# pashtari/lrf

Hardware: AMD Instinct MI355X
Metric: Mpixels/sec qmf_encode (8x8 patch, r=7, 10 iters) (higher is better)
Workload: dtype f32; 1 GPU; 256 x 512x768x3 uint8 per GPU, YCbCr 4:2:0, 8x8 patches, ranks (7,3,3), bounds (-16,15), num_iters 10, int8 factors out (BASELINE configs[1]); priming_steps=3, global_batch=256, rank_input_bytes=301989888, parallelism=images sharded over 1 GPU(s), no data-path collective

## Files before the change

lrf_amd/csrc/lrf_bcd_persist.hip:

```cpp
#include "lrf_host.h"
#include "lrf_gs.h"
#include "lrf_bcdw_kernel.hip"
#include "lrf_bcdw16_kernel.hip"
#include "lrf_bcdw32_kernel.hip"
#include "lrf_bcdp_kernel.hip"

PersistPlan bcdp_plan(lrf_ctx* c, const std::vector<FamRun>& runs, int K, int lo, int hi)
{
    PersistPlan pp;
    static const int persist_env = (int)env_long("LRF_PERSIST", -1);
    static const bool exact_off = dev_flag("LRF_GENERIC_GS");
    if (!c->persist_arch || persist_env == 0 || !bcd_wave_variant() || K < 2 || runs.empty()) return pp;
    const long mx = abs(lo) > abs(hi) ? abs(lo) : abs(hi);
    long nblocks = 0;
    bool f16 = false;
    int np32 = 0;
    for (const FamRun& r : runs) {
        if (fam_of_rank(r.rmin) != r.fam || fam_of_rank(r.rmax) != r.fam) return pp;
        nblocks += r.nblocks;
        if (r.fam == 0) continue;
        const bool exact = !exact_off && (long)(r.rmax - 1) * 64 * mx * mx * mx < (1L << 24);
        if (!exact || r.any_native) return pp;
        if (r.fam == 1) {
            f16 = true;
        } else {
            const int np = (r.rmax + 1) >> 1;
            if (64 * mx * mx > 32767 || r.rmin < 2 * np - 1 || (np32 != 0 && np32 != np)) return pp;
            np32 = np;
        }
    }
    const long min_blocks = runs.size() == 1 ? LRF_PERSIST_MIN_BLOCKS_ONE_FAMILY : LRF_PERSIST_MIN_BLOCKS;
    if (nblocks < (persist_env == 1 ? LRF_BCDW_MIN_BLOCKS : min_blocks)) return pp;
    pp.use = true;
    pp.f16 = f16 || np32 != 0;
    pp.np32 = np32;
    static const bool first_off = dev_flag("LRF_NO_PERSIST_FIRST");
    pp.first = np32 == 0 && !first_off;
    return pp;
}

template <bool F16, int NP32, bool FIRST = false>
static int bcdp_launch_t(lrf_ctx* c, int attr_bit, int wgs, int wave_lds, const float* X, const PlaneDesc* pl, const BlockDesc* bl, int nblocks,
                         int nplanes, int plane0, const BcdpTabs& t16, const BcdpTabs& t64, int8_t* U, int8_t* V, GsParams gp, int niter)
{
    if (!(c->attr_persist & (1u << attr_bit))) {
        HIP_TRY(hipFuncSetAttribute((const void*)k_bcd_p<F16, NP32, FIRST>, hipFuncAttributeMaxDynamicSharedMemorySize, LRF_BCDW_WAVES * wave_lds));
        c->attr_persist |= 1u << attr_bit;
    }
    Prof p(c, LRF_K_BCD_PERSIST);
    hipLaunchKernelGGL((k_bcd_p<F16, NP32, FIRST>), dim3((unsigned)wgs), dim3(64 * LRF_BCDW_WAVES), (size_t)LRF_BCDW_WAVES * wave_lds, c->stream, X, pl, bl, t16,
                       t64, U, V, gp, nblocks, niter, nplanes, plane0, (BcdpSync*)c->psync.p, c->h_perr, 2 * nplanes, ++c->pseq, wave_lds);
    LAUNCH_CHECK();
    return LRF_OK;
}

int bcdp_launch(lrf_ctx* c, const PersistPlan& pp, const float* X, const PlaneDesc* pl, const BlockDesc* bl, int nblocks, int nplanes, int plane0,
                const FamBufs& f16, const FamBufs& f64, int8_t* U, int8_t* V, GsParams gp, int niter, bool first)
{
    if (first && (!pp.first || pp.np32 != 0)) return set_err(LRF_EINVAL, "internal: first iteration inside k_bcd_p with ranks above 16");
    if (!c->h_perr) {
        HIP_TRY(hipHostMalloc((void**)&c->h_perr, sizeof(int), hipHostMallocDefault));
        *c->h_perr = 0;
    }
    int rc = ctx_check(c);
    if (rc) return rc;
    const size_t sbytes = sizeof(BcdpSync) + (2 * (size_t)nplanes + (size_t)nblocks) * sizeof(int);
    const void* before = c->psync.p;
    if ((rc = ensure(c, c->psync, sbytes))) return rc;
    if (c->psync.p != before || c->psync_dirty) {
        HIP_TRY(hipMemsetAsync(c->psync.p, 0, c->psync.cap, c->stream));
        c->psync_dirty = false;
    }
    const long total_waves = (long)niter * nblocks;
    long wgs = (total_waves + LRF_BCDW_WAVES - 1) / LRF_BCDW_WAVES;
    if (wgs > 512) wgs = 512;
    int wave_lds = (64 * 64 + 64 * 8) * 4;
    if (pp.f16 && LRF_BCDW16_WAVE_LDS > wave_lds) wave_lds = LRF_BCDW16_WAVE_LDS;
    const BcdpTabs t16{f16.vf, f16.bf, f16.pp, f16.qp, f16.wf}, t64{f64.vf, f64.bf, f64.pp, f64.qp, f64.wf};
    gp.exact_int = 1;
#define LRF_P(F16, NP, BIT)                                                                                                          \
    return bcdp_launch_t<F16, NP>(c, BIT, (int)wgs, NP ? (LRF_BCDW32_WAVE_LDS(NP) > wave_lds ? LRF_BCDW32_WAVE_LDS(NP) : wave_lds) : wave_lds, X, pl, bl, \
                                  nblocks, nplanes, plane0, t16, t64, U, V, gp, niter)
    if (first) {
        if (!pp.f16) return bcdp_launch_t<false, 0, true>(c, 10, (int)wgs, wave_lds, X, pl, bl, nblocks, nplanes, plane0, t16, t64, U, V, gp, niter);
        return bcdp_launch_t<true, 0, true>(c, 11, (int)wgs, wave_lds, X, pl, bl, nblocks, nplanes, plane0, t16, t64, U, V, gp, niter);
    }
    if (!pp.f16) LRF_P(false, 0, 0);
    switch (pp.np32) {
    case 0: LRF_P(true, 0, 1);
    case 9: LRF_P(true, 9, 2);
    case 10: LRF_P(true, 10, 3);
    case 11: LRF_P(true, 11, 4);
    case 12: LRF_P(true, 12, 5);
    case 13: LRF_P(true, 13, 6);
    case 14: LRF_P(true, 14, 7);
    case 15: LRF_P(true, 15, 8);
    default: LRF_P(true, 16, 9);
    }
#undef LRF_P
}
```

lrf_amd/csrc/lrf_bcdp_kernel.hip:

```cpp
#pragma once

#ifndef LRF_BCDP_MAX_POLLS
#define LRF_BCDP_MAX_POLLS (1 << 20)
#endif

struct BcdpSync {
    int head;
    int done;
    int err;
    int pad[29];
    int cell[1];
};

struct BcdpTabs {
    float *vf, *bf, *pp, *qp;
    const float* wf;
};

__device__ __forceinline__ float ld_sc1(const float* p) { return __hip_atomic_load(p, __ATOMIC_RELAXED, __HIP_MEMORY_SCOPE_AGENT); }
__device__ __forceinline__ void st_sc1(float* p, float v)
{
#ifdef LRF_BCDP_PLAIN_PSTORE
    *p = v;
#else
    __hip_atomic_store(p, v, __ATOMIC_RELAXED, __HIP_MEMORY_SCOPE_AGENT);
#endif
}
__device__ __forceinline__ void st_sc1_u32_unaligned(void* p, unsigned v)
{
#ifdef LRF_BCDP_PLAIN_USTORE
    *reinterpret_cast<u32_unaligned*>(p) = v;
#else
    asm volatile("global_store_dword %0, %1, off sc1" ::"v"(p), "v"(v) : "memory");
#endif
}
__device__ __forceinline__ unsigned ld_sc1_u32_unaligned(const void* p)
{
    unsigned v;
    asm volatile("global_load_dword %0, %1, off sc1" : "=v"(v) : "v"(p) : "memory");
    return v;
}

__device__ __forceinline__ void bcdp_sum16(const PlaneDesc& pd, const float* __restrict__ Ppart, const float* __restrict__ Qpart, int lane,
                                           float (&acc)[16], float (&q)[4])
{
#pragma unroll
    for (int j = 0; j < 16; j++) acc[j] = 0.f;
#pragma unroll
    for (int j = 0; j < 4; j++) q[j] = 0.f;
    const float* Pp = Ppart + (long)pd.blk0 * 64 * LRF_RP + lane;
    const float* Qp = Qpart + (long)pd.blk0 * LRF_RP * LRF_RP + lane;
    constexpr int NB = 4;
    for (int b0 = 0; b0 < pd.nblk; b0 += NB) {
        float pv[NB][16], qv[NB][4];
#pragma unroll
        for (int k = 0; k < NB; k++) {
            const long blk = b0 + k < pd.nblk ? b0 + k : b0;
#pragma unroll
            for (int j = 0; j < 16; j++) pv[k][j] = ld_sc1(Pp + blk * 64 * LRF_RP + 64 * j);
#pragma unroll
            for (int j = 0; j < 4; j++) qv[k][j] = ld_sc1(Qp + blk * LRF_RP * LRF_RP + 64 * j);
        }
#pragma unroll
        for (int k = 0; k < NB; k++)
            if (b0 + k < pd.nblk) {
#pragma unroll
                for (int j = 0; j < 16; j++) acc[j] = (b0 + k == 0) ? pv[k][j] : acc[j] + pv[k][j];
#pragma unroll
                for (int j = 0; j < 4; j++) q[j] = (b0 + k == 0) ? qv[k][j] : q[j] + qv[k][j];
            }
    }
}
__device__ __forceinline__ void bcdp_wave_sync()
{
    __builtin_amdgcn_fence(__ATOMIC_RELEASE, "wavefront");
    __builtin_amdgcn_wave_barrier();
    __builtin_amdgcn_fence(__ATOMIC_ACQUIRE, "wavefront");
}

__device__ __forceinline__ void bcdp_vupdate(const PlaneDesc& pd, int pli, const float* __restrict__ Ppart, const float* __restrict__ Qpart,
                                             float* __restrict__ Vf, float* __restrict__ Bf, int8_t* __restrict__ V8, const GsParams gp,
                                             int write_i8, float* lds, int lane)
{
    float* a_s = lds;
    float* v_s = lds + 64 * LRF_RP;
    float* gt_s = lds + 2 * 64 * LRF_RP;
    const int R = pd.R;
    float acc[16], q[4];
    bcdp_sum16(pd, Ppart, Qpart, lane, acc, q);
#pragma unroll
    for (int j = 0; j < 16; j++) {
        a_s[lane + 64 * j] = acc[j];
        v_s[lane + 64 * j] = ld_sc1(Vf + (long)pli * 64 * LRF_RP + lane + 64 * j);
    }
#pragma unroll
    for (int j = 0; j < 4; j++) {
        const int idx = lane + 64 * j, jj = idx >> 4, r = idx & 15;
        if (jj < R && r < R) {
            if (jj == r) {
                const float den = (q[j] + 0.f) + LRF_EPS;
                gt_s[r * LRF_GT_LD + LRF_GT_DEN] = den;
                gt_s[r * LRF_GT_LD + LRF_GT_RDEN] = 1.0f / den;
            } else {
                gt_s[r * LRF_GT_LD + (jj < r ? jj : jj - 1)] = q[j];
            }
        }
    }
    __builtin_amdgcn_fence(__ATOMIC_RELEASE, "wavefront");
    __builtin_amdgcn_wave_barrier();
    __builtin_amdgcn_fence(__ATOMIC_ACQUIRE, "wavefront");
    {
        const bool native = (long)(R - 1) * 64 < 400;
        const float no_tab[17] = {0.f, 0.f, 0.f, 0.f, 0.f, 0.f, 0.f, 0.f, 0.f, 0.f, 0.f, 0.f, 0.f, 0.f, 0.f, 0.f, 0.f};
        gs_dispatch<8, false>(R, &a_s[lane * LRF_RP], &v_s[lane * LRF_RP], nullptr, 0, gt_s, native, gp, no_tab);
        float* Vp = Vf + (long)pli * 64 * LRF_RP + lane * LRF_RP;
        for (int r = 0; r < R; r++) st_sc1(Vp + r, v_s[lane * LRF_RP + r]);
        if (write_i8) {
            int8_t* vo = V8 + pd.v_off + (long)lane * R;
            for (int r = 0; r < R; r++) vo[r] = (int8_t)v_s[lane * LRF_RP + r];
        }
    }
    __builtin_amdgcn_fence(__ATOMIC_RELEASE, "wavefront");
    __builtin_amdgcn_wave_barrier();
    __builtin_amdgcn_fence(__ATOMIC_ACQUIRE, "wavefront");
    if (!write_i8) {
        float* gt_n = a_s;
        make_gtable(v_s, 64, R, gt_n, lane, 64);
        __builtin_amdgcn_fence(__ATOMIC_RELEASE, "wavefront");
        __builtin_amdgcn_wave_barrier();
        __builtin_amdgcn_fence(__ATOMIC_ACQUIRE, "wavefront");
        float* gt_g = Bf + (long)pli * LRF_GT_STRIDE;
        for (int i = lane; i < R * LRF_GT_LD; i += 64) st_sc1(gt_g + i, gt_n[i]);
    }
}


__device__ __forceinline__ void bcdp_vupdate16(const PlaneDesc& pd, int pli, const float* __restrict__ Ppart, const float* __restrict__ Qpart,
                                               float* __restrict__ Vf, float* __restrict__ Bf, int8_t* __restrict__ V8, const GsParams gp,
                                               int write_i8, float* lds, int lane)
{
    float* a_s = lds;
    float* v_s = lds + 64 * LRF_RP;
    float* gt_b = lds + 2 * 64 * LRF_RP;
    const int R = pd.R;
    {
        float acc[16], q[4];
        bcdp_sum16(pd, Ppart, Qpart, lane, acc, q);
#pragma unroll
        for (int j = 0; j < 16; j++) {
            a_s[lane + 64 * j] = acc[j];
            v_s[lane + 64 * j] = ld_sc1(Vf + (long)pli * 64 * LRF_RP + lane + 64 * j);
        }
#pragma unroll
        for (int j = 0; j < 4; j++) {
            const int idx = lane + 64 * j, jj = idx >> 4, r = idx & 15;
            if (jj < R && r < R) {
                if (jj == r) gt_b[r * LRF_GTB_LD + LRF_GTB_DEN] = (q[j] + 0.f) + LRF_EPS;
                else gt_b[r * LRF_GTB_LD + (jj < r ? jj : jj - 1)] = q[j];
            }
        }
    }
    bcdp_wave_sync();
    {
        float a[32], v[32];
#pragma unroll
        for (int j = 0; j < 16; j += 4) {
            const f32x4 va4 = *reinterpret_cast<const f32x4*>(&a_s[lane * LRF_RP + j]);
            const f32x4 vv4 = *reinterpret_cast<const f32x4*>(&v_s[lane * LRF_RP + j]);
#pragma unroll
            for (int i = 0; i < 4; i++) { a[j + i] = va4[i]; v[j + i] = vv4[i]; }
        }
#pragma unroll
        for (int j = 16; j < 32; j++) a[j] = v[j] = 0.f;
        mid_ordered_row(R, a, v, gt_b, gp.lo, gp.hi, std::make_integer_sequence<int, 16>{});
        float* Vp = Vf + (long)pli * 64 * LRF_RP + lane * LRF_RP;
        int8_t* vo = V8 + pd.v_off + (long)lane * R;
#pragma unroll
        for (int r = 0; r < 16; r++)
            if (r < R) {
                v_s[lane * LRF_RP + r] = v[r];
                st_sc1(Vp + r, v[r]);
                if (write_i8) vo[r] = (int8_t)v[r];
            }
    }
    bcdp_wave_sync();
    if (!write_i8) {
        float* gt_n = a_s;
        make_gtable(v_s, 64, R, gt_n, lane, 64);
        bcdp_wave_sync();
        float* gt_g = Bf + (long)pli * LRF_GT_STRIDE;
        for (int i = lane; i < R * LRF_GT_LD; i += 64) st_sc1(gt_g + i, gt_n[i]);
    }
}

__device__ __forceinline__ void bcdp_vupdate32(const PlaneDesc& pd, int pli, const float* __restrict__ Ppart, const float* __restrict__ Qpart,
                                               float* __restrict__ Vf, float* __restrict__ Bf, int8_t* __restrict__ V8, const GsParams gp,
                                               int write_i8, float* lds, int lane)
{
    float* t_s = lds;
    float* gt_b = lds + 64 * 32;
    const int R = pd.R;
    float a[32], v[32];
    {
        float acc[32], q[16];
#pragma unroll
        for (int m = 0; m < 32; m++) acc[m] = 0.f;
#pragma unroll
        for (int m = 0; m < 16; m++) q[m] = 0.f;
        const float* P0 = Ppart + (long)pd.blk0 * 64 * LRF_RPB + (lane >> 5) * LRF_RPB + (lane & 31);
        const float* Q0 = Qpart + (long)pd.blk0 * LRF_RPB * LRF_RPB + (lane >> 5) * LRF_RPB + (lane & 31);
        constexpr int NB = 2;
        for (int b0 = 0; b0 < pd.nblk; b0 += NB) {
            float pv[NB][32], qv[NB][16];
#pragma unroll
            for (int k = 0; k < NB; k++) {
                const long blk = b0 + k < pd.nblk ? b0 + k : b0;
#pragma unroll
                for (int m = 0; m < 32; m++) pv[k][m] = ld_sc1(P0 + blk * 64 * LRF_RPB + 2 * m * LRF_RPB);
#pragma unroll
                for (int m = 0; m < 16; m++) qv[k][m] = ld_sc1(Q0 + blk * LRF_RPB * LRF_RPB + 2 * m * LRF_RPB);
            }
#pragma unroll
            for (int k = 0; k < NB; k++)
                if (b0 + k < pd.nblk) {
#pragma unroll
                    for (int m = 0; m < 32; m++) acc[m] = (b0 + k == 0) ? pv[k][m] : acc[m] + pv[k][m];
#pragma unroll
                    for (int m = 0; m < 16; m++) q[m] = (b0 + k == 0) ? qv[k][m] : q[m] + qv[k][m];
                }
        }
#pragma unroll
        for (int m = 0; m < 32; m++) t_s[lane + 64 * m] = acc[m];
#pragma unroll
        for (int m = 0; m < 16; m++) {
            const int j = 2 * m + (lane >> 5), r = lane & 31;
            if (j < R && r < R) {
                if (j == r) gt_b[r * LRF_GTB_LD + LRF_GTB_DEN] = (q[m] + 0.f) + LRF_EPS;
                else gt_b[r * LRF_GTB_LD + (j < r ? j : j - 1)] = q[m];
            }
        }
    }
    bcdp_wave_sync();
#pragma unroll
    for (int j = 0; j < 32; j += 4) {
        const f32x4 t4 = *reinterpret_cast<const f32x4*>(&t_s[lane * 32 + j]);
#pragma unroll
        for (int i = 0; i < 4; i++) a[j + i] = t4[i];
    }
    bcdp_wave_sync();
    {
        const float* Vg = Vf + (long)pli * 64 * LRF_RPB + (lane >> 5) * LRF_RPB + (lane & 31);
        float vv[32];
#pragma unroll
        for (int m = 0; m < 32; m++) vv[m] = ld_sc1(Vg + 2 * m * LRF_RPB);
#pragma unroll
        for (int m = 0; m < 32; m++) t_s[lane + 64 * m] = vv[m];
    }
    bcdp_wave_sync();
#pragma unroll
    for (int j = 0; j < 32; j += 4) {
        const f32x4 t4 = *reinterpret_cast<const f32x4*>(&t_s[lane * 32 + j]);
#pragma unroll
        for (int i = 0; i < 4; i++) v[j + i] = t4[i];
    }
    mid_ordered_row(R, a, v, gt_b, gp.lo, gp.hi, std::make_integer_sequence<int, 32>{});
    bcdp_wave_sync();
    {
        int8_t* vo = V8 + pd.v_off + (long)lane * R;
#pragma unroll
        for (int r = 0; r < 32; r++) {
            t_s[lane * 32 + r] = r < R ? v[r] : 0.f;
            if (write_i8 && r < R) vo[r] = (int8_t)v[r];
        }
    }
    bcdp_wave_sync();
    {
        float* Vg = Vf + (long)pli * 64 * LRF_RPB + (lane >> 5) * LRF_RPB + (lane & 31);
        if ((lane & 31) < R) {
#pragma unroll
            for (int m = 0; m < 32; m++) st_sc1(Vg + 2 * m * LRF_RPB, t_s[lane + 64 * m]);
        }
    }
    if (!write_i8) {
        float* gt_g = Bf + (long)pli * LRF_GTB_STRIDE;
        for (int i = lane; i < R * R; i += 64) {
            const int j = i / R, r = i - j * R;
            float acc = 0.f;
#pragma unroll 8
            for (int k = 0; k < 64; k++) acc = fmaf(t_s[k * 32 + j], t_s[k * 32 + r], acc);
            if (j == r) st_sc1(gt_g + r * LRF_GTB_LD + LRF_GTB_DEN, (acc + 0.f) + LRF_EPS);
            else st_sc1(gt_g + r * LRF_GTB_LD + (j < r ? j : j - 1), acc);
        }
    }
}

template <int MODE>
__device__ __forceinline__ void bcdp_w_block(const float* __restrict__ X, const PlaneDesc& pd, const BlockDesc& bd, const float* __restrict__ Vf,
                                             const float* __restrict__ Wf, const float* __restrict__ Bf, int8_t* __restrict__ U, float* __restrict__ Ppart,
                                             float* __restrict__ Qpart, const GsParams& gp, float* Xs, const int lane)
{
    constexpr int RMAX = 8;
    const int li = lane & 15, lq = lane >> 4;
    float* us = Xs + 64 * 64;
    const float* xp[4];
#pragma unroll
    for (int e = 0; e < 4; e++) xp[e] = &Xs[lq * 64 + 4 * (li ^ (4 * e + lq))];
    const float* ub = &us[lq * RMAX + (li & 7)];
    const float* uq = &us[(lq + 4 * (li >> 3)) * RMAX + (li & 7)];
    const float* xrow = &Xs[lane * 64];
    const int g16 = 16 * xsw(lane);
    const int R = pd.R;
    const float* Xp = X + pd.x_off + (long)bd.row0 * 64;
    const float* Vp = Vf + (long)bd.plane * 64 * LRF_RP;
    const float* gt = Bf + (long)bd.plane * LRF_GT_STRIDE;
    int8_t* Ub = U + pd.u_off + (long)bd.row0 * R;
    int nrows = pd.M - bd.row0;
    if (nrows > LRF_KC) nrows = LRF_KC;
    const int nsub = (nrows + 63) >> 6;
    const bool native = pd.native_t2_u != 0;

    float vreg[8][4], wreg[MODE == 1 ? 8 : 1][4];
#pragma unroll
    for (int r = 0; r < 8; r++)
#pragma unroll
        for (int kb = 0; kb < 4; kb++) {
            vreg[r][kb] = ld_sc1(Vp + (16 * kb + li) * LRF_RP + r);
            if constexpr (MODE == 1) wreg[r][kb] = Wf[((long)bd.plane * 64 + 16 * kb + li) * LRF_RP + r];
        }
    float tab[5];
#pragma unroll
    for (int j = 0; j < 4; j++) {
        const int ci = 16 * j + li, tr = ci >> 3, tn = ci & 7;
        tab[j] = ld_sc1(gt + tr * LRF_GT_LD + (tn < 7 ? tn : LRF_GT_RDEN));
    }
    tab[4] = ld_sc1(gt + (li & 7) * LRF_GT_LD + LRF_GT_DEN);

    f32x4 xq[4][4];
    auto issue_x = [&](int t, int T0, int T1, bool live) {
        const int r0 = t * 64;
#pragma unroll
        for (int T = T0; T < T1; T++) {
#pragma unroll
            for (int q = 0; q < 4; q++) {
                int row = r0 + 16 * T + 4 * q + lq;
                row = row < nrows ? row : nrows - 1;
                if (live) xq[T][q] = *reinterpret_cast<const f32x4*>(Xp + (long)row * 64 + 4 * li);
                else xq[T][q] = (f32x4){0.f, 0.f, 0.f, 0.f};
            }
        }
    };
    unsigned uraw[3];
    int ush = 0;
    auto issue_u = [&](int t) {
        int row = t * 64 + lane;
        row = row < nrows ? row : nrows - 1;
        const uintptr_t a0 = reinterpret_cast<uintptr_t>(Ub + (long)row * R);
        const uintptr_t base = a0 & ~(uintptr_t)3, last = (a0 + R - 1) & ~(uintptr_t)3;
        ush = (int)(a0 & 3);
        const unsigned* p0 = reinterpret_cast<const unsigned*>(base);
        const unsigned* p1 = reinterpret_cast<const unsigned*>(base + 4 <= last ? base + 4 : last);
        const unsigned* p2 = reinterpret_cast<const unsigned*>(base + 8 <= last ? base + 8 : last);
#ifdef LRF_BCDP_PLAIN_U
        uraw[0] = *p0; uraw[1] = *p1; uraw[2] = *p2;
#else
        uraw[0] = __hip_atomic_load(p0, __ATOMIC_RELAXED, __HIP_MEMORY_SCOPE_AGENT);
        uraw[1] = __hip_atomic_load(p1, __ATOMIC_RELAXED, __HIP_MEMORY_SCOPE_AGENT);
        uraw[2] = __hip_atomic_load(p2, __ATOMIC_RELAXED, __HIP_MEMORY_SCOPE_AGENT);
#endif
    };
    auto row_bytes = [&](unsigned& lo, unsigned& hi) {
        lo = __builtin_amdgcn_alignbyte(uraw[1], uraw[0], (unsigned)ush);
        hi = __builtin_amdgcn_alignbyte(uraw[2], uraw[1], (unsigned)ush);
    };

    f32x4 accP[4], accQ = (f32x4){0.f, 0.f, 0.f, 0.f};
#pragma unroll
    for (int c = 0; c < 4; c++) accP[c] = (f32x4){0.f, 0.f, 0.f, 0.f};

    if constexpr (MODE == 0) issue_u(0);
    issue_x(0, 0, 4, true);
    for (int t = 0; t < nsub; t++) {
        const int r0 = t * 64;
        __builtin_amdgcn_sched_barrier(0);
#pragma unroll
        for (int T = 0; T < 4; T++)
#pragma unroll
            for (int q = 0; q < 4; q++) {
                const int m = 16 * T + 4 * q + lq;
                *reinterpret_cast<f32x4*>(&Xs[m * 64 + 4 * (li ^ (4 * q + lq))]) = xq[T][q];
            }
        float u[RMAX];
        const int row = r0 + lane;
        if constexpr (MODE == 0) {
            unsigned lo, hi;
            row_bytes(lo, hi);
#pragma unroll
            for (int r = 0; r < 4; r++) {
                u[r] = (float)(int)(int8_t)(lo >> (8 * r));
                u[4 + r] = (float)(int)(int8_t)(hi >> (8 * r));
            }
        }
        const int tn = t + 1;
        const bool more = tn < nsub;
        if constexpr (MODE == 0) {
            if (more) issue_u(tn);
        }
        issue_x(tn, 0, 2, more);
        __builtin_amdgcn_fence(__ATOMIC_RELEASE, "wavefront");
        __builtin_amdgcn_wave_barrier();
        __builtin_amdgcn_fence(__ATOMIC_ACQUIRE, "wavefront");
        __builtin_amdgcn_sched_barrier(0);
        float a[RMAX];
#pragma unroll
        for (int r = 0; r < RMAX; r++) a[r] = 0.f;
        row_times_v_dispatch(R, xrow, g16, vreg, a);
        if constexpr (MODE == 1) {
#pragma unroll
            for (int r = 0; r < RMAX; r++) u[r] = 0.f;
            row_times_v_dispatch(R, xrow, g16, wreg, u);
        }
        issue_x(tn, 2, 3, more);
        __builtin_amdgcn_sched_barrier(0);
        gs_regs_dispatch<RMAX>(R, a, u, tab, native, gp);
        if (row >= nrows) {
#pragma unroll
            for (int r = 0; r < RMAX; r++) u[r] = 0.f;
        }
        issue_x(tn, 3, 4, more);
        __builtin_amdgcn_sched_barrier(0);
#pragma unroll
        for (int r = 0; r < RMAX; r += 4) *reinterpret_cast<f32x4*>(&us[lane * RMAX + r]) = (f32x4){u[r], u[r + 1], u[r + 2], u[r + 3]};
        if (row < nrows) {
            int8_t* uo = Ub + (long)row * R;
            unsigned lo = 0, hi = 0;
#pragma unroll
            for (int r = 0; r < 4; r++) {
                lo |= ((unsigned)(int)u[r] & 0xffu) << (8 * r);
                hi |= ((unsigned)(int)u[4 + r] & 0xffu) << (8 * r);
            }
            if (R >= 4) {
                st_sc1_u32_unaligned(uo, lo);
                const unsigned long long w = ((unsigned long long)hi << 32) | lo;
                st_sc1_u32_unaligned(uo + R - 4, (unsigned)(w >> (8 * (R - 4))));
            } else {
                __hip_atomic_store(uo, (int8_t)lo, __ATOMIC_RELAXED, __HIP_MEMORY_SCOPE_AGENT);
                if (R > 1) __hip_atomic_store(uo + 1, (int8_t)(lo >> 8), __ATOMIC_RELAXED, __HIP_MEMORY_SCOPE_AGENT);
                if (R > 2) __hip_atomic_store(uo + 2, (int8_t)(lo >> 16), __ATOMIC_RELAXED, __HIP_MEMORY_SCOPE_AGENT);
            }
        }
        __builtin_amdgcn_fence(__ATOMIC_RELEASE, "wavefront");
        __builtin_amdgcn_wave_barrier();
        __builtin_amdgcn_fence(__ATOMIC_ACQUIRE, "wavefront");
        __builtin_amdgcn_sched_barrier(0);
        float pu[16], qu[8];
#pragma unroll
        for (int s = 0; s < 16; s++) {
            float v = ub[4 * s * RMAX];
            pu[s] = (li < RMAX) ? v : 0.f;
        }
#pragma unroll
        for (int h = 0; h < 8; h++) qu[h] = uq[8 * h * RMAX];
        f32x4 px[16];
#pragma unroll
        for (int s = 0; s < 16; s++) px[s] = *reinterpret_cast<const f32x4*>(xp[s & 3] + 256 * s);
#pragma unroll
        for (int s = 0; s < 16; s++) {
#pragma unroll
            for (int c = 0; c < 4; c++) accP[c] = __builtin_amdgcn_mfma_f32_16x16x4f32(px[s][c], pu[s], accP[c], 0, 0, 0);
            if (s & 1) accQ = __builtin_amdgcn_mfma_f32_16x16x4f32(qu[s >> 1], qu[s >> 1], accQ, 0, 0, 0);
        }
        __builtin_amdgcn_sched_barrier(0);
        __builtin_amdgcn_fence(__ATOMIC_RELEASE, "wavefront");
        __builtin_amdgcn_wave_barrier();
        __builtin_amdgcn_fence(__ATOMIC_ACQUIRE, "wavefront");
    }
    const long slot = (long)pd.blk0 + bd.blk;
    float* Pp = Ppart + slot * 64 * LRF_RP;
#pragma unroll
    for (int c = 0; c < 4; c++)
#pragma unroll
        for (int reg = 0; reg < 4; reg++) st_sc1(Pp + (4 * (4 * lq + reg) + c) * LRF_RP + li, accP[c][reg]);
    float* Qp = Qpart + slot * LRF_RP * LRF_RP;
#pragma unroll
    for (int reg = 0; reg < 4; reg++) {
        const int i = 4 * lq + reg;
        const float mine = accQ[reg];
        const float other = __shfl(mine, ((lq + 2) & 3) * 16 + ((li + 8) & 15), 64);
        st_sc1(Qp + i * LRF_RP + li, (i < 8 && li < 8) ? mine + other : 0.f);
    }
}

template <bool F16, int NP32, bool FIRST = false>
__global__ __launch_bounds__(64 * LRF_BCDW_WAVES) __attribute__((amdgpu_waves_per_eu(2, 2))) void k_bcd_p(
    const float* __restrict__ X, const PlaneDesc* __restrict__ planes, const BlockDesc* __restrict__ blocks, const BcdpTabs t16,
    const BcdpTabs t64, int8_t* __restrict__ U, int8_t* __restrict__ V8, GsParams gp, int nblocks, int niter, int nplanes, int plane0,
    BcdpSync* sync, int* err_host, int ncells, int seq, int wave_lds)
{
    extern __shared__ __attribute__((aligned(16))) float bcdp_lds[];
    const int wave = __builtin_amdgcn_readfirstlane(threadIdx.x >> 6);
    const int lane = threadIdx.x & 63;
    float* Xs = reinterpret_cast<float*>(reinterpret_cast<char*>(bcdp_lds) + wave * wave_lds);
    int* ticket = sync->cell;
    int* flag = sync->cell + nplanes;
    const int total = niter * nblocks;
    auto leave = [&]() {
        asm volatile("s_waitcnt vmcnt(0)" ::: "memory");
        int l = 0;
        if (lane == 0) l = __hip_atomic_fetch_add(&sync->done, 1, __ATOMIC_RELAXED, __HIP_MEMORY_SCOPE_AGENT);
        const int d = __builtin_amdgcn_readfirstlane(__shfl(l, 0, 64));
        if (d == (int)(gridDim.x * LRF_BCDW_WAVES) - 1) {
            for (int i = lane; i < ncells; i += 64) __hip_atomic_store(&sync->cell[i], 0, __ATOMIC_RELAXED, __HIP_MEMORY_SCOPE_AGENT);
            __hip_atomic_store(&sync->head, 0, __ATOMIC_RELAXED, __HIP_MEMORY_SCOPE_AGENT);
            __hip_atomic_store(&sync->done, 0, __ATOMIC_RELAXED, __HIP_MEMORY_SCOPE_AGENT);
        }
    };

    if (__hip_atomic_load(&sync->err, __ATOMIC_RELAXED, __HIP_MEMORY_SCOPE_AGENT) != 0) return;
    for (;;) {
        int idx_l = 0;
        if (lane == 0) idx_l = __hip_atomic_fetch_add(&sync->head, 1, __ATOMIC_RELAXED, __HIP_MEMORY_SCOPE_AGENT);
        const int idx = __builtin_amdgcn_readfirstlane(__shfl(idx_l, 0, 64));
        if (idx >= total) {
            leave();
            return;
        }
        const int it = idx / nblocks, blk = idx - it * nblocks;
#ifdef LRF_BCDP_DEBUG
        atomicAdd(&sync->cell[2 * nplanes + blk], 1 + 1000 * it);
#endif
        const BlockDesc bd = blocks[blk];
        const PlaneDesc pd = planes[bd.plane];
        const int pl = bd.plane - plane0;
        if (it > 0) {
            int polls = 0;
            while (__hip_atomic_load(&flag[pl], __ATOMIC_RELAXED, __HIP_MEMORY_SCOPE_AGENT) < it) {
                __builtin_amdgcn_s_sleep(8);
                if (++polls > LRF_BCDP_MAX_POLLS) {
                    __hip_atomic_store(&sync->err, 1, __ATOMIC_RELAXED, __HIP_MEMORY_SCOPE_AGENT);
                    __hip_atomic_store(err_host, seq, __ATOMIC_RELAXED, __HIP_MEMORY_SCOPE_SYSTEM);
                    return;
                }
            }
        }
        __atomic_signal_fence(__ATOMIC_SEQ_CST);
        asm volatile("" ::: "memory");
#ifdef LRF_BCDP_FENCES
        __builtin_amdgcn_fence(__ATOMIC_ACQUIRE, "agent");
        asm volatile("s_waitcnt vmcnt(0)" ::: "memory");
#endif
        int ln = lane;
        asm volatile("" : "+v"(ln));
        const int fam = (!F16 || pd.R <= 8) ? 0 : ((NP32 == 0 || pd.R <= 16) ? 1 : 2);
        static_assert(!FIRST || NP32 == 0, "the first iteration of ranks 17..32 stays a launch of its own (k_bcd_w32f)");
        const bool first = FIRST && it == 0;
        if (fam == 0) {
            if (first) {
                if constexpr (FIRST) bcdp_w_block<1>(X, pd, bd, t16.vf, t16.wf, t16.bf, U, t16.pp, t16.qp, gp, Xs, ln);
            } else
                bcdp_w_block<0>(X, pd, bd, t16.vf, nullptr, t16.bf, U, t16.pp, t16.qp, gp, Xs, ln);
        }
        if constexpr (F16) {
            if (fam == 1) {
                if (first) {
                    if constexpr (FIRST) w16_block<1, MemSc1>(X, pd, bd, t16.vf, t16.wf, t16.bf, U, t16.pp, t16.qp, gp, Xs, ln);
                } else
                    w16_block<0, MemSc1>(X, pd, bd, t16.vf, nullptr, t16.bf, U, t16.pp, t16.qp, gp, Xs, ln);
            }
        }
        if constexpr (NP32 > 0) {
            if (fam == 2) w32_block<NP32, MemSc1>(X, pd, bd, t64.vf, t64.bf, U, t64.pp, t64.qp, gp, Xs, ln, 0);
        }
        asm volatile("s_waitcnt vmcnt(0)" ::: "memory");
#ifdef LRF_BCDP_FENCES
        __builtin_amdgcn_fence(__ATOMIC_RELEASE, "agent");
        asm volatile("s_waitcnt vmcnt(0)" ::: "memory");
#endif
        int arrived_l = 0;
        if (lane == 0) arrived_l = __hip_atomic_fetch_add(&ticket[pl], 1, __ATOMIC_RELAXED, __HIP_MEMORY_SCOPE_AGENT);
        const int arrived = __builtin_amdgcn_readfirstlane(__shfl(arrived_l, 0, 64));
        __atomic_signal_fence(__ATOMIC_SEQ_CST);
        asm volatile("" ::: "memory");
        if (arrived == (it + 1) * pd.nblk - 1) {
#ifdef LRF_BCDP_FENCES
            __builtin_amdgcn_fence(__ATOMIC_ACQUIRE, "agent");
            asm volatile("s_waitcnt vmcnt(0)" ::: "memory");
#endif
            const int last = it == niter - 1 ? 1 : 0;
            int lv = lane;
            asm volatile("" : "+v"(lv));
            if (fam == 0) bcdp_vupdate(pd, bd.plane, t16.pp, t16.qp, t16.vf, t16.bf, V8, gp, last, Xs, lv);
            if constexpr (F16) {
                if (fam == 1) bcdp_vupdate16(pd, bd.plane, t16.pp, t16.qp, t16.vf, t16.bf, V8, gp, last, Xs, lv);
            }
            if constexpr (NP32 > 0) {
                if (fam == 2) bcdp_vupdate32(pd, bd.plane, t64.pp, t64.qp, t64.vf, t64.bf, V8, gp, last, Xs, lv);
            }
            asm volatile("s_waitcnt vmcnt(0)" ::: "memory");
#ifdef LRF_BCDP_FENCES
            __builtin_amdgcn_fence(__ATOMIC_RELEASE, "agent");
            asm volatile("s_waitcnt vmcnt(0)" ::: "memory");
#endif
#ifdef LRF_BCDP_TEST_SKIP_FLAG
            if (!(pl == 0 && it == (FIRST ? 1 : 0) && niter == (FIRST ? 4 : 3)))
#endif
            __hip_atomic_store(&flag[pl], it + 1, __ATOMIC_RELAXED, __HIP_MEMORY_SCOPE_AGENT);
        }
    }
}
```

lrf_amd/csrc/lrf_device.h:

```cpp
#ifndef LRF_DEVICE_H
#define LRF_DEVICE_H
#include <hip/hip_runtime.h>
#include <stdint.h>

#include <utility>

#include "lrf_internal.h"

typedef int i32x4 __attribute__((ext_vector_type(4)));
typedef float f32x2 __attribute__((ext_vector_type(2)));
typedef unsigned __attribute__((aligned(1))) u32_unaligned;
typedef float f32x4 __attribute__((ext_vector_type(4)));
typedef double f64x4 __attribute__((ext_vector_type(4)));
typedef double d16 __attribute__((ext_vector_type(16)));

#define LRF_EPS 1e-16f
#define LRF_SIGMA_TINY 1e-280

#if defined(LRF_STAMPS) || defined(LRF_INIT_STAMPS) || defined(LRF_BLK_STAMPS) || defined(LRF_REG_STAMPS)
__device__ unsigned long long g_stamps[8 * 16384];
__device__ __forceinline__ unsigned long long stamp_now()
{
    unsigned long long t;
    __builtin_amdgcn_sched_barrier(0);
    asm volatile("s_memtime %0\n\ts_waitcnt lgkmcnt(0)" : "=s"(t)::"memory");
    __builtin_amdgcn_sched_barrier(0);
    return t;
}
#endif
#ifdef LRF_STAMPS
#define STAMP(var) unsigned long long var = stamp_now()
#define STAMP_ADD(acc, a, b) acc += (b) - (a)
__device__ unsigned long long g_gsp[4 * 16384];
#ifndef LRF_GS_PROBE
#define LRF_GS_PROBE 0
#endif
static constexpr int getenv_probe_dummy = LRF_GS_PROBE;
#define GSP_ADD(slot, a, b)                                                                     \
    if ((threadIdx.x & 63) == 0 && blockIdx.x < 16384) atomicAdd(&g_gsp[4 * blockIdx.x + (slot)], (b) - (a))
#else
#define STAMP(var)
#define STAMP_ADD(acc, a, b)
#define GSP_ADD(slot, a, b)
#endif

__device__ __forceinline__ int reflect_idx(int i, int n)
{
    if (i < 0) i = -i;
    if (i >= n) i = 2 * (n - 1) - i;
    return i;
}

__device__ __forceinline__ float ycc_of(float r, float g, float b, int c)
{
    const float T[3][3] = {{0.299f, 0.587f, 0.114f}, {-0.168736f, -0.331264f, 0.5f}, {0.5f, -0.418688f, -0.081312f}};
    float acc = 0.f;
    acc = fmaf(T[c][0], r, acc);
    acc = fmaf(T[c][1], g, acc);
    acc = fmaf(T[c][2], b, acc);
    return (c ? 128.f : 0.f) + acc;
}

__device__ __forceinline__ double partner_32(double v)
{
    int lo = __double2loint(v), hi = __double2hiint(v);
    auto a = __builtin_amdgcn_permlane32_swap(lo, lo, false, false);
    auto b = __builtin_amdgcn_permlane32_swap(hi, hi, false, false);
    return __hiloint2double(b[1], a[1]);
}
__device__ __forceinline__ double partner_16(double v)
{
    int lo = __double2loint(v), hi = __double2hiint(v);
    auto a = __builtin_amdgcn_permlane16_swap(lo, lo, false, false);
    auto b = __builtin_amdgcn_permlane16_swap(hi, hi, false, false);
    return __hiloint2double(b[1], a[1]);
}
template <int OFF>
__device__ __forceinline__ double partner_row(double v)
{
    int lo = __double2loint(v), hi = __double2hiint(v);
    lo = __builtin_amdgcn_update_dpp(0, lo, 0x100 + OFF, 0xf, 0xf, true);
    hi = __builtin_amdgcn_update_dpp(0, hi, 0x100 + OFF, 0xf, 0xf, true);
    return __hiloint2double(hi, lo);
}
__device__ __forceinline__ double wave_tree64(double v)
{
    v = v + partner_32(v);
    v = v + partner_16(v);
    v = v + partner_row<8>(v);
    v = v + partner_row<4>(v);
    v = v + partner_row<2>(v);
    v = v + partner_row<1>(v);
    int lo = __builtin_amdgcn_readfirstlane(__double2loint(v)), hi = __builtin_amdgcn_readfirstlane(__double2hiint(v));
    return __hiloint2double(hi, lo);
}

__device__ __forceinline__ void fmac_su(float& acc, float b_uniform, float u)
{
    asm("v_fmac_f32 %0, %1, %2" : "+v"(acc) : "s"(b_uniform), "v"(u));
}
template <int N>
__device__ __forceinline__ void fmac_bc16(float& acc, float tab, float x)
{
    asm("v_fmac_f32_dpp %0, %1, %2 row_newbcast:%3 row_mask:0xf bank_mask:0xf" : "+v"(acc) : "v"(tab), "v"(x), "n"(N));
}
template <int N>
__device__ __forceinline__ float get_bc16(float tab)
{
    float out;
    asm("v_mov_b32_dpp %0, %1 row_newbcast:%2 row_mask:0xf bank_mask:0xf" : "=v"(out) : "v"(tab), "n"(N));
    return out;
}

template <int N, class F>
__device__ __forceinline__ void static_for(F&& f)
{
    [&]<int... Is>(std::integer_sequence<int, Is...>) { (f(std::integral_constant<int, Is>{}), ...); }(std::make_integer_sequence<int, N>{});
}

struct MemLaunch {
    static constexpr bool kSc1 = false;
    static __device__ __forceinline__ float ld(const float* p) { return *p; }
    static __device__ __forceinline__ unsigned ld_u32(const unsigned* p) { return *p; }
    static __device__ __forceinline__ void st(float* p, float v) { *p = v; }
    static __device__ __forceinline__ void st_u32(void* p, unsigned v) { *reinterpret_cast<u32_unaligned*>(p) = v; }
    static __device__ __forceinline__ void st_u8(int8_t* p, int8_t v) { *p = v; }
};
struct MemSc1 {
    static constexpr bool kSc1 = true;
    static __device__ __forceinline__ float ld(const float* p) { return __hip_atomic_load(p, __ATOMIC_RELAXED, __HIP_MEMORY_SCOPE_AGENT); }
    static __device__ __forceinline__ unsigned ld_u32(const unsigned* p) { return __hip_atomic_load(p, __ATOMIC_RELAXED, __HIP_MEMORY_SCOPE_AGENT); }
    static __device__ __forceinline__ void st(float* p, float v) { __hip_atomic_store(p, v, __ATOMIC_RELAXED, __HIP_MEMORY_SCOPE_AGENT); }
    static __device__ __forceinline__ void st_u32(void* p, unsigned v)
    {
        asm volatile("global_store_dword %0, %1, off sc1" ::"v"(p), "v"(v) : "memory");
    }
    static __device__ __forceinline__ void st_u8(int8_t* p, int8_t v) { __hip_atomic_store(p, v, __ATOMIC_RELAXED, __HIP_MEMORY_SCOPE_AGENT); }
};
#endif
```

Measured before the change: 53760 Mpix/s.

## Vectorize persistent-kernel global traffic with 16-byte loads/stores and LDS-staged U rows

Replaces scalar coherent loads and stores in the persistent BCD kernel with 128-bit buffer loads and dwordx4 sc1 stores. U factor rows are staged through a new LDS region so a wave reads and writes contiguous 16-byte spans instead of per-row unaligned words. P/Q partial sums are packed densely (only R columns plus an RxR block) so the V-update reduction reads fewer bytes. Global pointers are also cast to the global address space so atomics lower to global rather than flat instructions. This adds LDS per wave and extra wave barriers, and the edge-store path has byte-granularity loops.

```diff
diff --git a/lrf_amd/csrc/lrf_bcd_persist.hip b/lrf_amd/csrc/lrf_bcd_persist.hip
--- a/lrf_amd/csrc/lrf_bcd_persist.hip
+++ b/lrf_amd/csrc/lrf_bcd_persist.hip
@@ -74,7 +74,7 @@
     const long total_waves = (long)niter * nblocks;
     long wgs = (total_waves + LRF_BCDW_WAVES - 1) / LRF_BCDW_WAVES;
     if (wgs > 512) wgs = 512;
-    int wave_lds = (64 * 64 + 64 * 8) * 4;
+    int wave_lds = (64 * 64 + 64 * 8) * 4 + LRF_BCDP_USTAGE;
     if (pp.f16 && LRF_BCDW16_WAVE_LDS > wave_lds) wave_lds = LRF_BCDW16_WAVE_LDS;
     const BcdpTabs t16{f16.vf, f16.bf, f16.pp, f16.qp, f16.wf}, t64{f64.vf, f64.bf, f64.pp, f64.qp, f64.wf};
     gp.exact_int = 1;
diff --git a/lrf_amd/csrc/lrf_bcdp_kernel.hip b/lrf_amd/csrc/lrf_bcdp_kernel.hip
--- a/lrf_amd/csrc/lrf_bcdp_kernel.hip
+++ b/lrf_amd/csrc/lrf_bcdp_kernel.hip
@@ -17,29 +17,31 @@
     const float* wf;
 };
 
-__device__ __forceinline__ float ld_sc1(const float* p) { return __hip_atomic_load(p, __ATOMIC_RELAXED, __HIP_MEMORY_SCOPE_AGENT); }
+__device__ __forceinline__ float ld_sc1(const float* p) { return __hip_atomic_load((const LRF_GLOBAL float*)p, __ATOMIC_RELAXED, __HIP_MEMORY_SCOPE_AGENT); }
 __device__ __forceinline__ void st_sc1(float* p, float v)
 {
 #ifdef LRF_BCDP_PLAIN_PSTORE
     *p = v;
 #else
-    __hip_atomic_store(p, v, __ATOMIC_RELAXED, __HIP_MEMORY_SCOPE_AGENT);
-#endif
-}
-__device__ __forceinline__ void st_sc1_u32_unaligned(void* p, unsigned v)
-{
-#ifdef LRF_BCDP_PLAIN_USTORE
-    *reinterpret_cast<u32_unaligned*>(p) = v;
-#else
-    asm volatile("global_store_dword %0, %1, off sc1" ::"v"(p), "v"(v) : "memory");
-#endif
-}
-__device__ __forceinline__ unsigned ld_sc1_u32_unaligned(const void* p)
-{
-    unsigned v;
-    asm volatile("global_load_dword %0, %1, off sc1" : "=v"(v) : "v"(p) : "memory");
-    return v;
-}
+    __hip_atomic_store((LRF_GLOBAL float*)p, v, __ATOMIC_RELAXED, __HIP_MEMORY_SCOPE_AGENT);
+#endif
+}
+typedef unsigned u32x4 __attribute__((ext_vector_type(4)));
+typedef unsigned u32x2 __attribute__((ext_vector_type(2)));
+__device__ __forceinline__ u32x4 ld_sc1_x4u(const void* base, unsigned off)
+{
+    const __amdgpu_buffer_rsrc_t rs = __builtin_amdgcn_make_buffer_rsrc(const_cast<void*>(base), (short)0, 0x7fffffff, 0x00020000);
+    return __builtin_bit_cast(u32x4, __builtin_amdgcn_raw_buffer_load_b128(rs, off, 0, 16));
+}
+__device__ __forceinline__ f32x4 ld_sc1_x4(const float* base, unsigned off) { return __builtin_bit_cast(f32x4, ld_sc1_x4u(base, off)); }
+__device__ __forceinline__ void st_sc1_x4(void* p, u32x4 v) { asm volatile("global_store_dwordx4 %0, %1, off sc1" ::"v"(p), "v"(v) : "memory"); }
+__device__ __forceinline__ void st_sc1_x2(void* p, u32x2 v) { asm volatile("global_store_dwordx2 %0, %1, off sc1" ::"v"(p), "v"(v) : "memory"); }
+__device__ __forceinline__ void st_sc1_b32(void* p, unsigned v) { asm volatile("global_store_dword %0, %1, off sc1" ::"v"(p), "v"(v) : "memory"); }
+__device__ __forceinline__ void st_sc1_b16(void* p, unsigned v) { asm volatile("global_store_short %0, %1, off sc1" ::"v"(p), "v"(v) : "memory"); }
+__device__ __forceinline__ void st_sc1_b8(void* p, unsigned v) { asm volatile("global_store_byte %0, %1, off sc1" ::"v"(p), "v"(v) : "memory"); }
+
+__device__ __forceinline__ int bcdp_dense_chunks(int R) { return (64 * R + R * R + 3) >> 2; }
+#define LRF_BCDP_USTAGE 544
 
 __device__ __forceinline__ void bcdp_sum16(const PlaneDesc& pd, const float* __restrict__ Ppart, const float* __restrict__ Qpart, int lane,
                                            float (&acc)[16], float (&q)[4])
@@ -78,31 +80,67 @@
     __builtin_amdgcn_fence(__ATOMIC_ACQUIRE, "wavefront");
 }
 
-__device__ __forceinline__ void bcdp_vupdate(const PlaneDesc& pd, int pli, const float* __restrict__ Ppart, const float* __restrict__ Qpart,
-                                             float* __restrict__ Vf, float* __restrict__ Bf, int8_t* __restrict__ V8, const GsParams gp,
-                                             int write_i8, float* lds, int lane)
+__device__ __forceinline__ void bcdp_sum_dense(const PlaneDesc& pd, const float* __restrict__ Ppart, int lane, float* sum_s)
+{
+    const int nch = bcdp_dense_chunks(pd.R), nj = (nch + 63) >> 6;
+    const float* base = Ppart + (long)pd.blk0 * 64 * LRF_RP;
+    f32x4 acc[3];
+#pragma unroll
+    for (int j = 0; j < 3; j++) acc[j] = (f32x4){0.f, 0.f, 0.f, 0.f};
+    constexpr int NB = 4;
+    for (int b0 = 0; b0 < pd.nblk; b0 += NB) {
+        f32x4 pv[NB][3];
+#pragma unroll
+        for (int k = 0; k < NB; k++) {
+            const unsigned blk = b0 + k < pd.nblk ? b0 + k : b0;
+#pragma unroll
+            for (int j = 0; j < 3; j++) {
+                const int c = lane + 64 * j < nch ? lane + 64 * j : nch - 1;
+                if (j < nj) pv[k][j] = ld_sc1_x4(base, (blk * 64 * LRF_RP + 4 * c) * 4);
+            }
+        }
+#pragma unroll
+        for (int k = 0; k < NB; k++)
+            if (b0 + k < pd.nblk) {
+#pragma unroll
+                for (int j = 0; j < 3; j++)
+                    if (j < nj) acc[j] = (b0 + k == 0) ? pv[k][j] : acc[j] + pv[k][j];
+            }
+    }
+#pragma unroll
+    for (int j = 0; j < 3; j++)
+        if (lane + 64 * j < nch) *reinterpret_cast<f32x4*>(&sum_s[4 * (lane + 64 * j)]) = acc[j];
+}
+
+__device__ __forceinline__ void bcdp_vupdate(const PlaneDesc& pd, int pli, const float* __restrict__ Ppart, float* __restrict__ Vf,
+                                             float* __restrict__ Bf, int8_t* __restrict__ V8, const GsParams gp, int write_i8, float* lds, int lane)
 {
     float* a_s = lds;
     float* v_s = lds + 64 * LRF_RP;
     float* gt_s = lds + 2 * 64 * LRF_RP;
+    float* sum_s = gt_s + LRF_GT_STRIDE;
     const int R = pd.R;
-    float acc[16], q[4];
-    bcdp_sum16(pd, Ppart, Qpart, lane, acc, q);
+    bcdp_sum_dense(pd, Ppart, lane, sum_s);
+    const float* Vg = Vf + (long)pli * 64 * LRF_RP;
+#pragma unroll
+    for (int j = 0; j < 4; j++) *reinterpret_cast<f32x4*>(&v_s[4 * (lane + 64 * j)]) = ld_sc1_x4(Vg, 16 * (lane + 64 * j));
+    bcdp_wave_sync();
 #pragma unroll
     for (int j = 0; j < 16; j++) {
-        a_s[lane + 64 * j] = acc[j];
-        v_s[lane + 64 * j] = ld_sc1(Vf + (long)pli * 64 * LRF_RP + lane + 64 * j);
+        const int idx = lane + 64 * j, n = idx >> 4, r = idx & 15;
+        a_s[idx] = r < R ? sum_s[r * 64 + n] : 0.f;
     }
 #pragma unroll
     for (int j = 0; j < 4; j++) {
         const int idx = lane + 64 * j, jj = idx >> 4, r = idx & 15;
         if (jj < R && r < R) {
+            const float q = sum_s[64 * R + jj * R + r];
             if (jj == r) {
-                const float den = (q[j] + 0.f) + LRF_EPS;
+                const float den = (q + 0.f) + LRF_EPS;
                 gt_s[r * LRF_GT_LD + LRF_GT_DEN] = den;
                 gt_s[r * LRF_GT_LD + LRF_GT_RDEN] = 1.0f / den;
             } else {
-                gt_s[r * LRF_GT_LD + (jj < r ? jj : jj - 1)] = q[j];
+                gt_s[r * LRF_GT_LD + (jj < r ? jj : jj - 1)] = q;
             }
         }
     }
@@ -130,7 +168,8 @@
         __builtin_amdgcn_wave_barrier();
         __builtin_amdgcn_fence(__ATOMIC_ACQUIRE, "wavefront");
         float* gt_g = Bf + (long)pli * LRF_GT_STRIDE;
-        for (int i = lane; i < R * LRF_GT_LD; i += 64) st_sc1(gt_g + i, gt_n[i]);
+        static_assert(LRF_GT_LD % 4 == 0, "the b table goes out in 16-B chunks");
+        for (int i = 4 * lane; i < R * LRF_GT_LD; i += 256) st_sc1_x4(gt_g + i, *reinterpret_cast<const u32x4*>(&gt_n[i]));
     }
 }
 
@@ -297,7 +336,7 @@
 template <int MODE>
 __device__ __forceinline__ void bcdp_w_block(const float* __restrict__ X, const PlaneDesc& pd, const BlockDesc& bd, const float* __restrict__ Vf,
                                              const float* __restrict__ Wf, const float* __restrict__ Bf, int8_t* __restrict__ U, float* __restrict__ Ppart,
-                                             float* __restrict__ Qpart, const GsParams& gp, float* Xs, const int lane)
+                                             const GsParams& gp, float* Xs, const int lane)
 {
     constexpr int RMAX = 8;
     const int li = lane & 15, lq = lane >> 4;
@@ -321,19 +360,31 @@
 
     float vreg[8][4], wreg[MODE == 1 ? 8 : 1][4];
 #pragma unroll
-    for (int r = 0; r < 8; r++)
-#pragma unroll
-        for (int kb = 0; kb < 4; kb++) {
-            vreg[r][kb] = ld_sc1(Vp + (16 * kb + li) * LRF_RP + r);
-            if constexpr (MODE == 1) wreg[r][kb] = Wf[((long)bd.plane * 64 + 16 * kb + li) * LRF_RP + r];
-        }
+    for (int kb = 0; kb < 4; kb++)
+#pragma unroll
+        for (int h = 0; h < 2; h++) {
+            const f32x4 v4 = ld_sc1_x4(Vp, ((16 * kb + li) * LRF_RP + 4 * h) * 4);
+#pragma unroll
+            for (int c = 0; c < 4; c++) vreg[4 * h + c][kb] = v4[c];
+        }
+    if constexpr (MODE == 1) {
+#pragma unroll
+        for (int r = 0; r < 8; r++)
+#pragma unroll
+            for (int kb = 0; kb < 4; kb++) wreg[r][kb] = Wf[((long)bd.plane * 64 + 16 * kb + li) * LRF_RP + r];
+    }
+    static_assert(LRF_GT_LD % 4 == 0 && LRF_GT_RDEN % 4 == 0 && LRF_GT_DEN == LRF_GT_RDEN + 1, "b-table chunks");
     float tab[5];
-#pragma unroll
-    for (int j = 0; j < 4; j++) {
-        const int ci = 16 * j + li, tr = ci >> 3, tn = ci & 7;
-        tab[j] = ld_sc1(gt + tr * LRF_GT_LD + (tn < 7 ? tn : LRF_GT_RDEN));
-    }
-    tab[4] = ld_sc1(gt + (li & 7) * LRF_GT_LD + LRF_GT_DEN);
+    {
+        const int tn = li & 7, e = tn < 7 ? (tn & 3) : 0;
+        f32x4 t4[5];
+#pragma unroll
+        for (int j = 0; j < 4; j++) t4[j] = ld_sc1_x4(gt, ((2 * j + (li >> 3)) * LRF_GT_LD + (tn < 7 ? (tn & 4) : LRF_GT_RDEN)) * 4);
+        t4[4] = ld_sc1_x4(gt, ((li & 7) * LRF_GT_LD + LRF_GT_RDEN) * 4);
+#pragma unroll
+        for (int j = 0; j < 4; j++) tab[j] = e == 0 ? t4[j][0] : e == 1 ? t4[j][1] : e == 2 ? t4[j][2] : t4[j][3];
+        tab[4] = t4[4][1];
+    }
 
     f32x4 xq[4][4];
     auto issue_x = [&](int t, int T0, int T1, bool live) {
@@ -349,28 +400,31 @@
             }
         }
     };
-    unsigned uraw[3];
-    int ush = 0;
+    uint8_t* ust = reinterpret_cast<uint8_t*>(Xs + 64 * 64 + 64 * RMAX);
+    const uintptr_t uaddr = reinterpret_cast<uintptr_t>(Ub);
+    const uint8_t* ub16 = reinterpret_cast<const uint8_t*>(uaddr & ~(uintptr_t)15);
+    auto span_of = [&](int t, uintptr_t& a, int& len, int& nsl) {
+        a = uaddr + (uintptr_t)(64 * R * t);
+        const int nr = nrows - 64 * t;
+        len = (nr < 64 ? nr : 64) * R;
+        nsl = ((int)(a & 15) + len + 15) >> 4;
+    };
+    u32x4 uvec;
+    int unsl = 0, uph = 0;
     auto issue_u = [&](int t) {
-        int row = t * 64 + lane;
-        row = row < nrows ? row : nrows - 1;
-        const uintptr_t a0 = reinterpret_cast<uintptr_t>(Ub + (long)row * R);
-        const uintptr_t base = a0 & ~(uintptr_t)3, last = (a0 + R - 1) & ~(uintptr_t)3;
-        ush = (int)(a0 & 3);
-        const unsigned* p0 = reinterpret_cast<const unsigned*>(base);
-        const unsigned* p1 = reinterpret_cast<const unsigned*>(base + 4 <= last ? base + 4 : last);
-        const unsigned* p2 = reinterpret_cast<const unsigned*>(base + 8 <= last ? base + 8 : last);
-#ifdef LRF_BCDP_PLAIN_U
-        uraw[0] = *p0; uraw[1] = *p1; uraw[2] = *p2;
-#else
-        uraw[0] = __hip_atomic_load(p0, __ATOMIC_RELAXED, __HIP_MEMORY_SCOPE_AGENT);
-        uraw[1] = __hip_atomic_load(p1, __ATOMIC_RELAXED, __HIP_MEMORY_SCOPE_AGENT);
-        uraw[2] = __hip_atomic_load(p2, __ATOMIC_RELAXED, __HIP_MEMORY_SCOPE_AGENT);
-#endif
+        uintptr_t a;
+        int len;
+        span_of(t, a, len, unsl);
+        uph = (int)(a & 15);
+        const int k = lane < unsl ? lane : unsl - 1;
+        uvec = ld_sc1_x4u(ub16, (unsigned)((a & ~(uintptr_t)15) - reinterpret_cast<uintptr_t>(ub16)) + 16 * k);
     };
-    auto row_bytes = [&](unsigned& lo, unsigned& hi) {
-        lo = __builtin_amdgcn_alignbyte(uraw[1], uraw[0], (unsigned)ush);
-        hi = __builtin_amdgcn_alignbyte(uraw[2], uraw[1], (unsigned)ush);
+    auto row_bytes = [&](int ph, unsigned& lo, unsigned& hi) {
+        const int o = ph + lane * R;
+        const unsigned* w = reinterpret_cast<const unsigned*>(ust + (o & ~3));
+        const unsigned w0 = w[0], w1 = w[1], w2 = w[2];
+        lo = __builtin_amdgcn_alignbyte(w1, w0, (unsigned)(o & 3));
+        hi = __builtin_amdgcn_alignbyte(w2, w1, (unsigned)(o & 3));
     };
 
     f32x4 accP[4], accQ = (f32x4){0.f, 0.f, 0.f, 0.f};
@@ -391,14 +445,10 @@
             }
         float u[RMAX];
         const int row = r0 + lane;
+        int cph = 0;
         if constexpr (MODE == 0) {
-            unsigned lo, hi;
-            row_bytes(lo, hi);
-#pragma unroll
-            for (int r = 0; r < 4; r++) {
-                u[r] = (float)(int)(int8_t)(lo >> (8 * r));
-                u[4 + r] = (float)(int)(int8_t)(hi >> (8 * r));
-            }
+            if (lane < unsl) *reinterpret_cast<u32x4*>(ust + 16 * lane) = uvec;
+            cph = uph;
         }
         const int tn = t + 1;
         const bool more = tn < nsub;
@@ -409,6 +459,15 @@
         __builtin_amdgcn_fence(__ATOMIC_RELEASE, "wavefront");
         __builtin_amdgcn_wave_barrier();
         __builtin_amdgcn_fence(__ATOMIC_ACQUIRE, "wavefront");
+        if constexpr (MODE == 0) {
+            unsigned lo, hi;
+            row_bytes(cph, lo, hi);
+#pragma unroll
+            for (int r = 0; r < 4; r++) {
+                u[r] = (float)(int)(int8_t)(lo >> (8 * r));
+                u[4 + r] = (float)(int)(int8_t)(hi >> (8 * r));
+            }
+        }
         __builtin_amdgcn_sched_barrier(0);
         float a[RMAX];
 #pragma unroll
@@ -430,27 +489,45 @@
         __builtin_amdgcn_sched_barrier(0);
 #pragma unroll
         for (int r = 0; r < RMAX; r += 4) *reinterpret_cast<f32x4*>(&us[lane * RMAX + r]) = (f32x4){u[r], u[r + 1], u[r + 2], u[r + 3]};
+        uintptr_t sa;
+        int slen, snsl;
+        span_of(t, sa, slen, snsl);
+        const int sph = (int)(sa & 15);
         if (row < nrows) {
-            int8_t* uo = Ub + (long)row * R;
-            unsigned lo = 0, hi = 0;
-#pragma unroll
-            for (int r = 0; r < 4; r++) {
-                lo |= ((unsigned)(int)u[r] & 0xffu) << (8 * r);
-                hi |= ((unsigned)(int)u[4 + r] & 0xffu) << (8 * r);
-            }
-            if (R >= 4) {
-                st_sc1_u32_unaligned(uo, lo);
-                const unsigned long long w = ((unsigned long long)hi << 32) | lo;
-                st_sc1_u32_unaligned(uo + R - 4, (unsigned)(w >> (8 * (R - 4))));
-            } else {
-                __hip_atomic_store(uo, (int8_t)lo, __ATOMIC_RELAXED, __HIP_MEMORY_SCOPE_AGENT);
-                if (R > 1) __hip_atomic_store(uo + 1, (int8_t)(lo >> 8), __ATOMIC_RELAXED, __HIP_MEMORY_SCOPE_AGENT);
-                if (R > 2) __hip_atomic_store(uo + 2, (int8_t)(lo >> 16), __ATOMIC_RELAXED, __HIP_MEMORY_SCOPE_AGENT);
-            }
+            uint8_t* d = ust + sph + lane * R;
+#pragma unroll
+            for (int r = 0; r < RMAX; r++)
+                if (r < R) d[r] = (uint8_t)(int)u[r];
         }
         __builtin_amdgcn_fence(__ATOMIC_RELEASE, "wavefront");
         __builtin_amdgcn_wave_barrier();
         __builtin_amdgcn_fence(__ATOMIC_ACQUIRE, "wavefront");
+        if (lane < snsl) {
+            const uintptr_t s0 = (sa & ~(uintptr_t)15) + 16 * lane;
+            const uint8_t* src = ust + 16 * lane;
+            int lo = lane == 0 ? sph : 0;
+            const int hi = lane == snsl - 1 ? sph + slen - 16 * lane : 16;
+            if (lo == 0 && hi == 16) {
+                st_sc1_x4(reinterpret_cast<void*>(s0), *reinterpret_cast<const u32x4*>(src));
+            } else {
+                while (lo < hi) {
+                    void* dst = reinterpret_cast<void*>(s0 + lo);
+                    if ((lo & 7) == 0 && lo + 8 <= hi) {
+                        st_sc1_x2(dst, *reinterpret_cast<const u32x2*>(src + lo));
+                        lo += 8;
+                    } else if ((lo & 3) == 0 && lo + 4 <= hi) {
+                        st_sc1_b32(dst, *reinterpret_cast<const unsigned*>(src + lo));
+                        lo += 4;
+                    } else if ((lo & 1) == 0 && lo + 2 <= hi) {
+                        st_sc1_b16(dst, *reinterpret_cast<const uint16_t*>(src + lo));
+                        lo += 2;
+                    } else {
+                        st_sc1_b8(dst, src[lo]);
+                        lo += 1;
+                    }
+                }
+            }
+        }
         __builtin_amdgcn_sched_barrier(0);
         float pu[16], qu[8];
 #pragma unroll
@@ -474,20 +551,25 @@
         __builtin_amdgcn_wave_barrier();
         __builtin_amdgcn_fence(__ATOMIC_ACQUIRE, "wavefront");
     }
-    const long slot = (long)pd.blk0 + bd.blk;
-    float* Pp = Ppart + slot * 64 * LRF_RP;
-#pragma unroll
-    for (int c = 0; c < 4; c++)
-#pragma unroll
-        for (int reg = 0; reg < 4; reg++) st_sc1(Pp + (4 * (4 * lq + reg) + c) * LRF_RP + li, accP[c][reg]);
-    float* Qp = Qpart + slot * LRF_RP * LRF_RP;
+    float* ps = Xs;
+    if (li < R) {
+#pragma unroll
+        for (int reg = 0; reg < 4; reg++)
+            *reinterpret_cast<f32x4*>(&ps[li * 64 + 16 * lq + 4 * reg]) = (f32x4){accP[0][reg], accP[1][reg], accP[2][reg], accP[3][reg]};
+    }
 #pragma unroll
     for (int reg = 0; reg < 4; reg++) {
         const int i = 4 * lq + reg;
         const float mine = accQ[reg];
         const float other = __shfl(mine, ((lq + 2) & 3) * 16 + ((li + 8) & 15), 64);
-        st_sc1(Qp + i * LRF_RP + li, (i < 8 && li < 8) ? mine + other : 0.f);
-    }
+        if (i < R && li < R) ps[64 * R + i * R + li] = mine + other;
+    }
+    __builtin_amdgcn_fence(__ATOMIC_RELEASE, "wavefront");
+    __builtin_amdgcn_wave_barrier();
+    __builtin_amdgcn_fence(__ATOMIC_ACQUIRE, "wavefront");
+    float* Pp = Ppart + ((long)pd.blk0 + bd.blk) * 64 * LRF_RP;
+    const int nch = bcdp_dense_chunks(R);
+    for (int c = lane; c < nch; c += 64) st_sc1_x4(Pp + 4 * c, *reinterpret_cast<const u32x4*>(&ps[4 * c]));
 }
 
 template <bool F16, int NP32, bool FIRST = false>
@@ -555,9 +637,9 @@
         const bool first = FIRST && it == 0;
         if (fam == 0) {
             if (first) {
-                if constexpr (FIRST) bcdp_w_block<1>(X, pd, bd, t16.vf, t16.wf, t16.bf, U, t16.pp, t16.qp, gp, Xs, ln);
+                if constexpr (FIRST) bcdp_w_block<1>(X, pd, bd, t16.vf, t16.wf, t16.bf, U, t16.pp, gp, Xs, ln);
             } else
-                bcdp_w_block<0>(X, pd, bd, t16.vf, nullptr, t16.bf, U, t16.pp, t16.qp, gp, Xs, ln);
+                bcdp_w_block<0>(X, pd, bd, t16.vf, nullptr, t16.bf, U, t16.pp, gp, Xs, ln);
         }
         if constexpr (F16) {
             if (fam == 1) {
@@ -588,7 +670,7 @@
             const int last = it == niter - 1 ? 1 : 0;
             int lv = lane;
             asm volatile("" : "+v"(lv));
-            if (fam == 0) bcdp_vupdate(pd, bd.plane, t16.pp, t16.qp, t16.vf, t16.bf, V8, gp, last, Xs, lv);
+            if (fam == 0) bcdp_vupdate(pd, bd.plane, t16.pp, t16.vf, t16.bf, V8, gp, last, Xs, lv);
             if constexpr (F16) {
                 if (fam == 1) bcdp_vupdate16(pd, bd.plane, t16.pp, t16.qp, t16.vf, t16.bf, V8, gp, last, Xs, lv);
             }
diff --git a/lrf_amd/csrc/lrf_device.h b/lrf_amd/csrc/lrf_device.h
--- a/lrf_amd/csrc/lrf_device.h
+++ b/lrf_amd/csrc/lrf_device.h
@@ -126,15 +126,19 @@
     static __device__ __forceinline__ void st_u32(void* p, unsigned v) { *reinterpret_cast<u32_unaligned*>(p) = v; }
     static __device__ __forceinline__ void st_u8(int8_t* p, int8_t v) { *p = v; }
 };
+#define LRF_GLOBAL __attribute__((address_space(1)))
 struct MemSc1 {
     static constexpr bool kSc1 = true;
-    static __device__ __forceinline__ float ld(const float* p) { return __hip_atomic_load(p, __ATOMIC_RELAXED, __HIP_MEMORY_SCOPE_AGENT); }
-    static __device__ __forceinline__ unsigned ld_u32(const unsigned* p) { return __hip_atomic_load(p, __ATOMIC_RELAXED, __HIP_MEMORY_SCOPE_AGENT); }
-    static __device__ __forceinline__ void st(float* p, float v) { __hip_atomic_store(p, v, __ATOMIC_RELAXED, __HIP_MEMORY_SCOPE_AGENT); }
+    static __device__ __forceinline__ float ld(const float* p) { return __hip_atomic_load((const LRF_GLOBAL float*)p, __ATOMIC_RELAXED, __HIP_MEMORY_SCOPE_AGENT); }
+    static __device__ __forceinline__ unsigned ld_u32(const unsigned* p)
+    {
+        return __hip_atomic_load((const LRF_GLOBAL unsigned*)p, __ATOMIC_RELAXED, __HIP_MEMORY_SCOPE_AGENT);
+    }
+    static __device__ __forceinline__ void st(float* p, float v) { __hip_atomic_store((LRF_GLOBAL float*)p, v, __ATOMIC_RELAXED, __HIP_MEMORY_SCOPE_AGENT); }
     static __device__ __forceinline__ void st_u32(void* p, unsigned v)
     {
         asm volatile("global_store_dword %0, %1, off sc1" ::"v"(p), "v"(v) : "memory");
     }
-    static __device__ __forceinline__ void st_u8(int8_t* p, int8_t v) { __hip_atomic_store(p, v, __ATOMIC_RELAXED, __HIP_MEMORY_SCOPE_AGENT); }
+    static __device__ __forceinline__ void st_u8(int8_t* p, int8_t v) { __hip_atomic_store((LRF_GLOBAL int8_t*)p, v, __ATOMIC_RELAXED, __HIP_MEMORY_SCOPE_AGENT); }
 };
 #endif
```

After: 56040 Mpix/s (median of 6 runs). 4.2% higher.
